# xingyizhou/CenterTrack

Measured on AMD Instinct MI355X. Metric: frames/sec (DLA-34 + DCNv2 CenterTrack hot path: H2D of the frame + forward + decode + D2H + track association), higher is better.
Workload: dtype f32; 1 GPU; mot17_512: mot heads, DLA-34, 512x512, 1 stream(s)/GPU, K=100, flip_test=False, seeded random-init weights; one step = 64 consecutive frames of every stream, each frame uploaded from pinned host memory inside the step (frame t+1 on a copy stream while frame t runs); global_batch=1, parallelism=streams sharded dp1, all-gather of packed detections, hip_graph=True

## Files before the change

### centertrack_amd/_lib.py

```python
import ctypes
import os

_PKG = os.path.dirname(os.path.abspath(__file__))
LIB_PATH = os.environ.get('CENTERTRACK_LIB') or os.path.join(_PKG, 'libcentertrack_hip.so')

c_float_p = ctypes.c_void_p
NUM_HEADS = 11
(HEAD_REG, HEAD_WH, HEAD_TRACKING, HEAD_LTRB, HEAD_LTRB_AMODAL, HEAD_DEP, HEAD_ROT, HEAD_DIM,
 HEAD_AMODEL_OFFSET, HEAD_NUSCENES_ATT, HEAD_VELOCITY) = range(NUM_HEADS)
HEAD_INDEX = {'reg': HEAD_REG, 'wh': HEAD_WH, 'tracking': HEAD_TRACKING, 'ltrb': HEAD_LTRB,
              'ltrb_amodal': HEAD_LTRB_AMODAL, 'dep': HEAD_DEP, 'rot': HEAD_ROT, 'dim': HEAD_DIM,
              'amodel_offset': HEAD_AMODEL_OFFSET, 'nuscenes_att': HEAD_NUSCENES_ATT,
              'velocity': HEAD_VELOCITY}
HEAD_CH = {'reg': 2, 'wh': 2, 'tracking': 2, 'ltrb': 4, 'ltrb_amodal': 4, 'dep': 1, 'rot': 8, 'dim': 3,
           'amodel_offset': 2, 'nuscenes_att': 8, 'velocity': 3}

CT_RELU = 1
CT_OUT_NCHW = 2
CT_DCN_MAIN, CT_DCN_FINISH, CT_DCN_OFFSETS = 1, 2, 4
CT_OK, CT_ERR_ARG, CT_ERR_LAUNCH, CT_ERR_WORKSPACE = 0, 1, 2, 3


class ConvDesc(ctypes.Structure):
    _fields_ = [('x', ctypes.c_void_p), ('N', ctypes.c_int), ('H', ctypes.c_int), ('W', ctypes.c_int),
                ('Cin', ctypes.c_int), ('ldx', ctypes.c_int),
                ('w_packed', ctypes.c_void_p), ('Cout', ctypes.c_int), ('ks', ctypes.c_int),
                ('stride', ctypes.c_int),
                ('scale', ctypes.c_void_p), ('shift', ctypes.c_void_p),
                ('res', ctypes.c_void_p), ('ldr', ctypes.c_int),
                ('y', ctypes.c_void_p), ('ldy', ctypes.c_int),
                ('flags', ctypes.c_int),
                ('sig_lo', ctypes.c_int), ('sig_hi', ctypes.c_int),
                ('dep_lo', ctypes.c_int), ('dep_hi', ctypes.c_int), ('depth_scale', ctypes.c_float),
                ('workspace', ctypes.c_void_p), ('workspace_bytes', ctypes.c_size_t),
                ('split_k', ctypes.c_int), ('algo', ctypes.c_int), ('w_winograd', ctypes.c_void_p),
                ('pool_y', ctypes.c_void_p), ('pool_ld', ctypes.c_int),
                ('proj_w_packed', ctypes.c_void_p), ('proj_scale', ctypes.c_void_p), ('proj_shift', ctypes.c_void_p),
                ('proj_y', ctypes.c_void_p), ('proj_ldy', ctypes.c_int)]


class DcnDesc(ctypes.Structure):
# ... 274 lines not shown
```

### centertrack_amd/build.py

```python
import os
import subprocess
import sys

PKG = os.path.dirname(os.path.abspath(__file__))
ROOT = os.path.dirname(PKG)
CSRC = os.path.join(PKG, 'csrc')
LIB = os.path.join(PKG, 'libcentertrack_hip.so')
SOURCES = ['api.cpp', 'runtime.hip', 'conv_mfma.hip', 'wino_mfma.hip', 'dcn_mfma.hip', 'stem.hip', 'elementwise.hip', 'decode.hip', 'pose.hip', 'host_track.cpp', 'host_preprocess.cpp', 'preprocess.hip', 'flip.hip', 'frame_loop.hip']
FLAGS = ['--offload-arch=gfx950', '-O3', '-std=c++17', '-fPIC', '-I' + os.path.join(ROOT, 'include'), '-I' + CSRC,
         '-Wno-unused-result']


def _stale(target, deps):
    if not os.path.exists(target):
        return True
    t = os.path.getmtime(target)
    return any(os.path.getmtime(d) > t for d in deps)


def build(force=False, verbose=False):
    hipcc = os.environ.get('HIPCC', '/opt/rocm/bin/hipcc')
    objdir = os.path.join(PKG, 'build')
    os.makedirs(objdir, exist_ok=True)
    headers = [os.path.join(CSRC, 'ct_common.h'), os.path.join(CSRC, 'ksplit_core.h'),
               os.path.join(ROOT, 'include', 'centertrack_hip.h')]
    objs = []
    procs = []
    for src in SOURCES:
        sp = os.path.join(CSRC, src)
        if not os.path.exists(sp):
            continue
        obj = os.path.join(objdir, src.rsplit('.', 1)[0] + '.o')
        objs.append(obj)
        if force or _stale(obj, [sp] + headers):
            extra = ['-x', 'hip'] if src.endswith('.hip') else ['-ffp-contract=off']
            cmd = [hipcc] + FLAGS + extra + ['-c', sp, '-o', obj]
            if verbose:
                print(' '.join(cmd))
            procs.append((src, subprocess.Popen(cmd)))
    for src, p in procs:
        if p.wait() != 0:
            raise RuntimeError('hipcc failed on %s' % src)
    if force or _stale(LIB, objs):
        cmd = [hipcc, '--offload-arch=gfx950', '-shared', '-fPIC', '-pthread', '-o', LIB] + objs
        if verbose:
            print(' '.join(cmd))
        subprocess.check_call(cmd)
# ... 6 lines not shown
```

### centertrack_amd/csrc/ct_common.h

```cpp
#pragma once
#include <hip/hip_runtime.h>
#include <stdint.h>
#include <stdio.h>

#include "centertrack_hip.h"

typedef float f32x4 __attribute__((ext_vector_type(4)));

void ct_set_error(const char *fmt, ...);

#define CT_FAIL_ARG(...)            \
    do {                            \
        ct_set_error(__VA_ARGS__);  \
        return CT_ERR_ARG;          \
    } while (0)

#define CT_CHECK_LAUNCH(name)                                              \
    do {                                                                   \
        hipError_t e__ = hipGetLastError();                                \
        if (e__ != hipSuccess) {                                           \
            ct_set_error("%s: launch failed: %s", name, hipGetErrorString(e__)); \
            return CT_ERR_LAUNCH;                                          \
        }                                                                  \
    } while (0)

static inline int ct_cdiv(int a, int b) { return (a + b - 1) / b; }

enum { CT_TUNE_CONV_CFG = 0, CT_TUNE_CONV_PIPE, CT_TUNE_CONV_SMALL_TILES, CT_TUNE_SPLITK_TARGET, CT_TUNE_DCN_BN,
       CT_TUNE_CONV_KS, CT_TUNE_CONV_KS_BELOW, CT_TUNE_CONV_KS_WAVES, CT_TUNE_XCD_REMAP, CT_TUNE_HEADS_ORDER, CT_TUNE_STEM_ROWS, CT_TUNE_DCN_SLOTS, CT_TUNE_DCN_XCD, CT_TUNE_COUNT };
int ct_tune_get(int key);
void ct_affine_inverse(const double *trans, double *M);
struct ct_wino_off_layer {
    const float *x; int N, H, W, Cin, ldx;
    const float *w_winograd;
    float *part;
};
int ct_wino_offsets_group(const ct_wino_off_layer *layers, int n, void *stream);

static inline int ct_xcd_per(int coutBlocks)
{
    return (ct_tune_get(CT_TUNE_XCD_REMAP) && coutBlocks >= 16 && (coutBlocks & 7) == 0) ? (coutBlocks >> 3) : 0;
}
#ifdef __HIPCC__
__device__ __forceinline__ int ct_block_cout(int &bid, int coutBlocks, int per)
{
    int cb;
    if (per) {
        const int j = bid >> 3;
        cb = (bid & 7) + 8 * (j % per);
        bid = j / per;
    } else {
        cb = bid % coutBlocks;
        bid /= coutBlocks;
    }
    return cb;
}
#endif

// ... 123 lines not shown
```

### centertrack_amd/csrc/dcn_mfma.hip

```cpp
#include <type_traits>

#include "ct_common.h"
#include "ksplit_core.h"

namespace {

struct DcnArgs {
    const float *x;
    const float *om;
    const float *wp;
    int N, H, W, Cin, ldx, ldom;
    int tilesX, tilesY, coutBlocks;
    int NT;
    int nchunks, chunksPerSplit;
    int tiles;
    int ptiles, splits;
    int xsx, xper, pband;
    float *ws;
    int wsCout;
    const float *w_off;
    const float *b_off;
    float *omPart;
    int omSplits;
    int offsOnly;
    EpiArgs epi;
};

constexpr int DCN_MAX_GROUP = 4;
struct DcnGroup {
    DcnArgs p[DCN_MAX_GROUP];
    int first[DCN_MAX_GROUP + 1];
    int n;
};

#ifndef CT_OFF_PD
#define CT_OFF_PD 2
#endif
CT_DEFINE_STAMPS(dcn)
#ifndef CT_ABL
#define CT_ABL 0
#endif
#ifndef CT_WS_AUX
#define CT_WS_AUX 0
#endif

__device__ __forceinline__ float dcn_mask_sigmoid(float v) { return __builtin_amdgcn_rcpf(1.0f + __expf(-v)); }

typedef float f32x2 __attribute__((ext_vector_type(2)));
__device__ __forceinline__ f32x4 dcn_blend(const f32x4 w, const f32x4 (&c)[4])
{
    const f32x2 w01 = w.lo, w23 = w.hi;
    f32x2 lo, hi;
    asm("v_pk_mul_f32 %0, %1, %2 op_sel_hi:[0,1]" : "=v"(lo) : "v"(w01), "v"(c[0].lo));
    asm("v_pk_mul_f32 %0, %1, %2 op_sel_hi:[0,1]" : "=v"(hi) : "v"(w01), "v"(c[0].hi));
    asm("v_pk_fma_f32 %0, %1, %2, %0 op_sel:[1,0,0] op_sel_hi:[1,1,1]" : "+v"(lo) : "v"(w01), "v"(c[1].lo));
    asm("v_pk_fma_f32 %0, %1, %2, %0 op_sel:[1,0,0] op_sel_hi:[1,1,1]" : "+v"(hi) : "v"(w01), "v"(c[1].hi));
    asm("v_pk_fma_f32 %0, %1, %2, %0 op_sel_hi:[0,1,1]" : "+v"(lo) : "v"(w23), "v"(c[2].lo));
    asm("v_pk_fma_f32 %0, %1, %2, %0 op_sel_hi:[0,1,1]" : "+v"(hi) : "v"(w23), "v"(c[2].hi));
    asm("v_pk_fma_f32 %0, %1, %2, %0 op_sel:[1,0,0] op_sel_hi:[1,1,1]" : "+v"(lo) : "v"(w23), "v"(c[3].lo));
    asm("v_pk_fma_f32 %0, %1, %2, %0 op_sel:[1,0,0] op_sel_hi:[1,1,1]" : "+v"(hi) : "v"(w23), "v"(c[3].hi));
    return f32x4{lo[0], lo[1], hi[0], hi[1]};
}

__device__ __forceinline__ void dcn_tab_entry(float dy, float dx, float mk, float fyk, float fxk, bool in, int H, int W, int ldx4,
                                              int rowb, int4 &o, f32x4 &w)
{
    const float ys = fyk + dy, xs = fxk + dx;
    const float yf = floorf(ys), xf = floorf(xs);
    const int y0 = (int)yf, x0 = (int)xf;
    const float ly = ys - yf, lx = xs - xf, hy = 1.0f - ly, hx = 1.0f - lx;
    const bool ok = in & (ys > -1.0f) & (xs > -1.0f) & (ys < (float)H) & (xs < (float)W);
    const bool vy0 = ok & (y0 >= 0), vy1 = ok & (y0 + 1 <= H - 1), vx0 = x0 >= 0, vx1 = x0 + 1 <= W - 1;
    const int base = __mul24(__mul24(y0, W) + x0, ldx4);
    o.x = (vy0 & vx0) ? base : 0;
    o.y = (vy0 & vx1) ? base + ldx4 : 0;
    o.z = (vy1 & vx0) ? base + rowb : 0;
    o.w = (vy1 & vx1) ? base + rowb + ldx4 : 0;
    w[0] = (vy0 & vx0) ? hy * hx * mk : 0.0f;
    w[1] = (vy0 & vx1) ? hy * lx * mk : 0.0f;
    w[2] = (vy1 & vx0) ? ly * hx * mk : 0.0f;
    w[3] = (vy1 & vx1) ? ly * lx * mk : 0.0f;
}

template <int WM, int WN>
__device__ __forceinline__ void dcn_store_acc(const DcnArgs &a, const f32x4 (&acc)[WM][WN], int n, int oy0, int ox0, int split, int nt0,
                                              int wm, int lane, const float (&psc)[WN], const float (&psh)[WN])
{
    const int li = lane & 15, lg = lane >> 4;
    if (a.ws) {
        const size_t Mtot = (size_t)a.N * a.H * a.W;
        float *wsp = a.ws + (size_t)split * Mtot * a.wsCout;
        const __amdgpu_buffer_rsrc_t srs = __builtin_amdgcn_make_buffer_rsrc(wsp, 0, (int)(Mtot * a.wsCout * 4), 0x00020000);
        const int pixb = a.wsCout * 4, rowb2 = a.W * pixb;
        const int oyb = oy0 + wm * WM;
        const int px0 = ox0 + lg * 4;
#pragma unroll
        for (int nt = 0; nt < WN; ++nt) {
            const int co = (nt0 + nt) * 16 + li;
            const int vbase = (((n * a.H + oyb) * a.W + px0) * a.wsCout + co) * 4;
            int vo[4];
#pragma unroll
            for (int e = 0; e < 4; ++e) vo[e] = (co < a.wsCout && px0 + e < a.W) ? vbase : (int)0x80000000;
#pragma unroll
            for (int mt = 0; mt < WM; ++mt) {
// ... 138 lines not shown
                b[kk][nt] = __builtin_bit_cast(f32x4, __builtin_amdgcn_raw_buffer_load_b128(wrs, bvo[nt], so + kk * slab_bytes, 0));
    };
    const int nsteps = (c_end - c_begin) * 9;
    const int nmax = nsteps;
    auto step_ct = [&](int st, int &chunk, int &tap) {
        const int u = min(max(st, 0), max(nsteps - 1, 0));
        const int c = u / 9;
        chunk = min(c_begin + c, nunits - 1);
        tap = u - c * 9;
    };
    f32x4 bq[2][NKK][WN];
    {
        int ch, tp;
        step_ct(0, ch, tp);
        load_b(bq[0], ch, tp);
    }
    float psc[WN], psh[WN];
#pragma unroll
    for (int nt = 0; nt < WN; ++nt) {
        psc[nt] = 1.0f; psh[nt] = 0.0f;
        if (!a.ws) ct_load_scale_shift(a.epi, (nt0 + nt) * 16, lane, psc[nt], psh[nt]);
    }

    {
        constexpr int E = BM * 9;
        constexpr int TI = (E + NTHR - 1) / NTHR;
        const int ldx4 = a.ldx * 4, rowb = a.W * ldx4;
        float tdy[TI], tdx[TI], tmk[TI];
        const int rot = (blockIdx.x >> 8) & 3;
        const int wrot = (wave - rot) & 3, trot = (tid - rot * 64) & 255;
#pragma unroll
        for (int i = 0; i < TI; ++i) {
            if (wrot * 64 + NTHR * i >= E) continue;
            const int it = trot + NTHR * i;
            const int k = it / BM, m = it & (BM - 1);
            const int oy = oy0 + (m >> 4), ox = ox0 + (m & 15);
            const bool in = it < E && oy < a.H && ox < a.W;
            if (parts) {
                const size_t plane = (size_t)a.N * a.H * a.W * 32;
                const float *pp = a.omPart + (in ? (((size_t)n * a.H + oy) * a.W + ox) * 32 : 0);
                const int kk = in ? k : 0;
                float dy = pp[2 * kk], dx = pp[2 * kk + 1], mk = pp[18 + kk];
                for (int sp = 1; sp < a.omSplits; ++sp) {
                    dy += pp[sp * plane + 2 * kk];
                    dx += pp[sp * plane + 2 * kk + 1];
                    mk += pp[sp * plane + 18 + kk];
// ... 432 lines not shown
    }
    CT_STAMP_VAL(17, nsteps);
    CT_STAMP_VAL(18, pi);
    CT_STAMP_RT(15);
}

}

extern "C" size_t ct_dcn_v2_offsets_bytes(const ct_dcn_desc *d)
{
    if (!d || (d->fuse_offset != 2 && d->fuse_offset != 3) || d->Cin % 64 || d->Cin <= 0 || d->N <= 0 || d->H <= 0 || d->W <= 0)
        return 0;
    return (size_t)(d->fuse_offset == 3 ? 1 : d->Cin / 64) * d->N * d->H * d->W * 32 * sizeof(float);
}

namespace {

struct DcnPlan {
    int fuse;
    int parts;
    int BM, BN, NKK, tilesX, tilesY, coutBlocks, NT, nchunks, splits, chunksPerSplit;
    int use_ws;
    int persist;
};

int make_plan(const ct_dcn_desc *d, DcnPlan *p, bool grouped)
{
    if (!d || !d->x || !d->w_packed || !d->y) CT_FAIL_ARG("ct_dcn_v2: null pointer");
    if (d->fuse_offset < 0 || d->fuse_offset > 3) CT_FAIL_ARG("ct_dcn_v2: fuse_offset=%d (0 .. 3)", d->fuse_offset);
    p->fuse = d->fuse_offset == 1;
    p->parts = d->fuse_offset == 2 ? d->Cin / 64 : (d->fuse_offset == 3 ? 1 : 0);
    if (d->fuse_offset && (!d->b_off || (d->fuse_offset != 3 && !d->w_off_packed && !(d->fuse_offset == 2 && d->w_off_winograd))))
        CT_FAIL_ARG("ct_dcn_v2: fuse_offset needs w_off_packed and b_off");
    if (d->fuse_offset && d->Cin % 64) CT_FAIL_ARG("ct_dcn_v2: fuse_offset needs Cin %% 64 == 0 (got %d)", d->Cin);
    if (p->parts) {
        const size_t need = ct_dcn_v2_offsets_bytes(d);
        if (!d->om_partial || d->om_partial_bytes < need) {
            ct_set_error("ct_dcn_v2: fuse_offset=%d needs %zu bytes of om_partial, got %zu", d->fuse_offset, need, d->om_partial ? d->om_partial_bytes : (size_t)0);
            return CT_ERR_WORKSPACE;
        }
    }
    if (!d->fuse_offset && !d->om) CT_FAIL_ARG("ct_dcn_v2: null offset/mask map");
    if (d->up_w) {
        if (!d->up_skip || !d->up_y) CT_FAIL_ARG("ct_dcn_v2: up_w given without up_skip / up_y");
        if (d->up_f != 2 && d->up_f != 4 && d->up_f != 8) CT_FAIL_ARG("ct_dcn_v2: up_f=%d unsupported", d->up_f);
        if (d->Cout % 4 || d->up_lds % 4 || d->up_ldy % 4 || ((uintptr_t)d->up_skip & 15) || ((uintptr_t)d->up_y & 15))
            CT_FAIL_ARG("ct_dcn_v2: up-sample views must be 16-byte aligned with Cout %% 4 == 0");
// ... 38 lines not shown
    }
    if (p->NKK == 4 && d->Cin % 64) CT_FAIL_ARG("ct_dcn_v2: the 64-channel-step shapes need Cin %% 64 == 0 (got %d)", d->Cin);
    p->tilesY = ct_cdiv(d->H, p->BM / 16);
    p->coutBlocks = ct_cdiv(d->Cout, p->BN);
    p->nchunks = d->Cin / 32;
    const long tiles = (long)d->N * p->tilesX * p->tilesY * p->coutBlocks;
    int splits = d->split_k;
    if (splits <= 0) {
        splits = 1;
        if (grouped) {
            splits = p->nchunks / 2;
        } else if (d->workspace && tiles < 256) {
            splits = (int)((512 + tiles - 1) / tiles);
            if (splits > 16) splits = 16;
        }
    }
    const int upc = p->NKK / 2;
    const int nunits = p->nchunks / upc;
    if (splits > nunits) splits = nunits;
    if (splits < 1) splits = 1;
    p->chunksPerSplit = ct_cdiv(nunits, splits) * upc;
    p->splits = ct_cdiv(p->nchunks, p->chunksPerSplit);
    p->use_ws = (p->splits > 1 || (grouped && d->up_w)) ? 1 : 0;
    if (p->persist) {
        const int ups = p->chunksPerSplit / upc;
        if (p->BM != 32 || (ups & 1) || nunits % ups)
            CT_FAIL_ARG("ct_dcn_v2: persistent shape needs an even number of %d-channel units per split (Cin=%d, split_k=%d)", 16 * p->NKK, d->Cin, p->splits);
        if ((double)d->N * d->H * d->W * d->ldx * 4.0 >= 4294967296.0) CT_FAIL_ARG("ct_dcn_v2: persistent shape: input view of 4 GiB or more");
    }
    return CT_OK;
}

size_t ws_bytes(const ct_dcn_desc *d, const DcnPlan &p)
{
    if (!p.use_ws) return 0;
    return (size_t)p.splits * d->N * d->H * d->W * (size_t)(p.NT * 16) * sizeof(float);
}

struct UpArgs {
    const float *w;
    const float *skip;
    float *y;
    int f, lds, ldy;
};
struct RedArgs {
    const float *ws;
    int splits, wsCout;
    size_t Mtot;
    int N, H, W;
    int rowBlocks;
    EpiArgs e;
    UpArgs u;
};
struct RedGroup {
    RedArgs p[DCN_MAX_GROUP];
    int first[DCN_MAX_GROUP + 1];
    int n;
};

// ... 55 lines not shown
        for (int jx = 0; jx < 2; ++jx) {
            const int xx = ix - jx;
            if (xx < 0 || xx >= W) continue;
            const unsigned m = ((unsigned)n * H + yy) * W + xx;
            const float *src = ws + (size_t)(m * wsCout + c);
            f32x4 s = *reinterpret_cast<const f32x4 *>(src);
            for (int k = 1; k < splits; ++k) s += *reinterpret_cast<const f32x4 *>(src + (size_t)k * plane);
            const int widx = (ky + f * jy) * kw + (kx + f * jx);
            const f32x4 wv = *reinterpret_cast<const f32x4 *>(u.w + widx * C + c);
#pragma unroll
            for (int i = 0; i < 4; ++i) acc[i] += ct_epilogue_value(e, s[i], c + i, sc[i], sh[i], 0.0f) * wv[i];
        }
    }
    *reinterpret_cast<f32x4 *>(u.y + (size_t)opix * u.ldy + c) = acc;
}

void fill_args(const ct_dcn_desc *d, const DcnPlan &p, DcnArgs *a)
{
    a->x = d->x; a->om = d->om; a->wp = d->w_packed;
    a->N = d->N; a->H = d->H; a->W = d->W; a->Cin = d->Cin; a->ldx = d->ldx; a->ldom = d->ldom;
    a->tilesX = p.tilesX; a->tilesY = p.tilesY; a->coutBlocks = p.coutBlocks; a->NT = p.NT;
    a->nchunks = p.nchunks; a->chunksPerSplit = p.chunksPerSplit;
    a->tiles = d->N * p.tilesX * p.tilesY * p.coutBlocks;
    a->ws = p.use_ws ? d->workspace : nullptr;
    a->wsCout = p.NT * 16;
    a->epi.scale = d->scale; a->epi.shift = d->shift; a->epi.res = nullptr; a->epi.y = d->y;
    a->epi.ldr = 0; a->epi.ldy = d->ldy; a->epi.Cout = d->Cout; a->epi.Ho = d->H; a->epi.Wo = d->W;
    a->epi.flags = d->flags & CT_RELU; a->epi.sig_lo = a->epi.sig_hi = 0; a->epi.dep_lo = a->epi.dep_hi = 0;
    a->epi.depth_scale = 1.0f;
    a->w_off = p.fuse ? d->w_off_packed : nullptr;
    a->b_off = d->fuse_offset ? d->b_off : nullptr;
    a->omPart = p.parts ? d->om_partial : nullptr;
    a->omSplits = p.parts;
    a->offsOnly = 0;
    a->ptiles = d->N * p.tilesX * p.tilesY;
    a->splits = p.splits;
    a->xsx = 0; a->xper = 0; a->pband = 0;
    if (ct_tune_get(CT_TUNE_DCN_XCD)) {
        int sx = 1;
        while (sx < 8 && p.splits % (2 * sx) == 0) sx *= 2;
        a->xsx = sx;
        a->pband = ct_cdiv(a->ptiles, 8 / sx);
        a->xper = p.coutBlocks * (p.splits / sx) * a->pband;
    }
}

size_t lds_bytes(int BM, bool fuse_any, bool single_chunk, int NKK = 2)
{
    using OffCfg = KsCfg<3, 1, 2, 2, 4>;
    size_t regionA = sizeof(float) * (size_t)(2 * NKK * BM * 16 + 2 * BM * 9 * 4);
    if (!fuse_any) return regionA;
    const size_t scratch = single_chunk ? sizeof(float) * (size_t)OffCfg::LDS1_FLOATS : OffCfg::LDS_BYTES;
    return sizeof(float) * (size_t)(BM * 32) + (scratch > regionA ? scratch : regionA);
}

int launch_group(const ct_dcn_desc *descs, int n, bool grouped, int phases, void *stream)
{
// ... 6 lines not shown
    long blocks = 0, rblocks = 0;
    bool fuse_any = false, single_chunk = true;
    const ct_dcn_desc *legacy_up = nullptr;
    for (int i = 0; i < n; ++i) {
        const ct_dcn_desc *d = descs + i;
        DcnPlan &p = plans[i];
        int rc = make_plan(d, &p, grouped);
        if (rc != CT_OK) return rc;
        if ((phases & CT_DCN_MAIN) && (p.BM != plans[0].BM || p.BN != plans[0].BN || p.NKK != plans[0].NKK || p.persist != plans[0].persist))
            CT_FAIL_ARG("ct_dcn_v2_group: layer %d resolves to another tile shape than layer 0", i);
        const size_t need = ws_bytes(d, p);
        if (need > 0 && (!d->workspace || d->workspace_bytes < need)) {
            ct_set_error("ct_dcn_v2: layer %d: split_k=%d needs %zu workspace bytes, got %zu", i, p.splits, need, d->workspace_bytes);
            return CT_ERR_WORKSPACE;
        }
        fill_args(d, p, &g.p[i]);
        fuse_any = fuse_any || p.fuse;
        if (p.fuse && d->Cin != 64) single_chunk = false;
        g.first[i] = (int)blocks;
        blocks += g.p[i].xsx ? 8L * g.p[i].xper : (long)g.p[i].tiles * p.splits;
        if (blocks > 0x7fffffffL) CT_FAIL_ARG("ct_dcn_v2: grid too large");
        if (p.use_ws) {
            RedArgs &r = rg.p[rg.n];
            r.ws = d->workspace; r.splits = p.splits; r.wsCout = g.p[i].wsCout;
            r.Mtot = (size_t)d->N * d->H * d->W;
            r.N = d->N; r.H = d->H; r.W = d->W;
            r.e = g.p[i].epi;
            long rows;
            if (d->up_w) {
                r.u.w = d->up_w; r.u.skip = d->up_skip; r.u.y = d->up_y; r.u.f = d->up_f; r.u.lds = d->up_lds; r.u.ldy = d->up_ldy;
                r.rowBlocks = (d->W * d->up_f * (d->Cout / 4) + 255) / 256;
                rows = (long)d->N * d->H * d->up_f;
            } else {
                r.u.w = nullptr; r.u.skip = nullptr; r.u.y = nullptr; r.u.f = 0; r.u.lds = r.u.ldy = 0;
                r.rowBlocks = (d->W * (r.wsCout / 4) + 255) / 256;
                rows = (long)d->N * d->H;
            }
            if ((double)r.Mtot * r.wsCout >= 1073741824.0 ||
                (d->up_w && (double)r.Mtot * d->up_f * d->up_f * (d->up_lds > d->up_ldy ? d->up_lds : d->up_ldy) >= 4294967296.0))
                CT_FAIL_ARG("ct_dcn_v2: layer %d: partial map / IDAUp output too large for the finishing launch", i);
            rg.first[rg.n] = (int)rblocks;
            rblocks += rows * r.rowBlocks;
            if (rblocks > 0x7fffffffL) CT_FAIL_ARG("ct_dcn_v2: grid too large");
            ++rg.n;
        } else if (d->up_w) {
            legacy_up = d;
        }
    }
    g.first[n] = (int)blocks;
    for (int i = n + 1; i <= DCN_MAX_GROUP; ++i) g.first[i] = (int)blocks;
    for (int i = n; i < DCN_MAX_GROUP; ++i) g.p[i] = g.p[0];
    const DcnPlan &p0 = plans[0];
    hipStream_t s = (hipStream_t)stream;
    if (phases & CT_DCN_OFFSETS) {
        DcnGroup og;
        og.n = 0;
        long oblocks = 0;
        ct_wino_off_layer wl[DCN_MAX_GROUP];
        int nw = 0;
        for (int i = 0; i < n; ++i) {
            const ct_dcn_desc *d = descs + i;
            if (d->fuse_offset != 2) continue;
            if (d->w_off_winograd) {
                ct_wino_off_layer &l = wl[nw++];
                l.x = d->x; l.N = d->N; l.H = d->H; l.W = d->W; l.Cin = d->Cin; l.ldx = d->ldx;
                l.w_winograd = d->w_off_winograd; l.part = d->om_partial;
                continue;
            }
            DcnArgs &a = og.p[og.n];
            a = g.p[i];
            a.tilesX = ct_cdiv(d->W, 16); a.tilesY = ct_cdiv(d->H, 2); a.coutBlocks = 1;
            a.tiles = d->N * a.tilesX * a.tilesY;
            a.w_off = d->w_off_packed;
            a.offsOnly = 1;
            og.first[og.n] = (int)oblocks;
            oblocks += (long)a.tiles * plans[i].parts;
            ++og.n;
        }
        if (og.n > 0) {
            if (oblocks > 0x7fffffffL) CT_FAIL_ARG("ct_dcn_v2: grid too large");
            for (int i = og.n; i <= DCN_MAX_GROUP; ++i) og.first[i] = (int)oblocks;
            for (int i = og.n; i < DCN_MAX_GROUP; ++i) og.p[i] = og.p[0];
            hipLaunchKernelGGL((dcn_mfma_kernel<32, 1, true>), dim3((unsigned)oblocks), dim3(256), lds_bytes(32, true, true), s, og);
            CT_CHECK_LAUNCH("ct_dcn_v2(offset/mask conv)");
        }
        if (nw > 0) {
            const int rc = ct_wino_offsets_group(wl, nw, stream);
            if (rc != CT_OK) return rc;
        }
// ... 135 lines not shown
```

### centertrack_amd/csrc/wino_mfma.hip

```cpp
#include "ct_common.h"

typedef unsigned u32x4 __attribute__((ext_vector_type(4)));

namespace {

struct WinoArgs {
    const float *x;
    const float *up;
    int N, H, W, Cin, ldx;
    int tilesX, tilesY, coutBlocks, xcdPer;
    int headMajor;
    int NT;
    int nchunks;
    EpiArgs epi;
    const float *hw2;
    const float *hb2;
    float *hout;
    int hctot;
    int hcout[CT_MAX_FUSED_HEADS], hcoff[CT_MAX_FUSED_HEADS];
};

template <int WM>
struct WCfg {
    static constexpr int PH = 4 * WM + 2, PW = 18, PP = PH * PW;
// ... 421 lines not shown
                    const float v = (hacc[h2][j] + hred[((q * 64 + lane) * 2 + h2) * 8 + j]) + a.hb2[cb * 8 + j];
                    a.hout[(((size_t)n * a.hctot + gc) * a.epi.Ho + oy) * a.epi.Wo + ox] =
                        ct_epilogue_value(a.epi, v, gc, 1.0f, 0.0f, 0.0f);
                }
            }
        }
    }
    if (HEADS) { CT_STAMP(6); CT_STAMP_RT(7); }
}

template <int WM, int WN, int KS, bool MULTI, int NB = 1, bool HEADS = false>
__global__ __launch_bounds__(256 * KS)
__attribute__((amdgpu_waves_per_eu(NB > 1 ? CT_NB_WAVES : ((!MULTI && KS == 1 && WM * WN <= 2) ? 4 : KS))))
void wino_conv_kernel(WinoArgs a)
{
    wino_body<WM, WN, KS, MULTI, NB, HEADS>(a, (int)blockIdx.x, gridDim.x, 0, a.epi.y);
}

struct WinoGroup {
    WinoArgs p[4];
    int first[5];
    int tiles[4];
    int sx[4], pband[4];
    int n;
};

__global__ __launch_bounds__(256) __attribute__((amdgpu_waves_per_eu(4))) void wino_offsets_kernel(WinoGroup g)
{
    int bid = blockIdx.x;
    int pi = 0;
#pragma unroll
    for (int i = 1; i < 4; ++i)
        if (i < g.n && bid >= g.first[i]) pi = i;
    const WinoArgs a = g.p[pi];
    bid -= g.first[pi];
    const int tiles = g.tiles[pi];
    const int sx = g.sx[pi], sper = (a.Cin >> 6) / sx;
    const int xcd = bid & 7;
    int j = bid >> 3;
    const int sh = j % sper; j /= sper;
    const int split = (xcd & (sx - 1)) + sx * sh;
    bid = (xcd / sx) * g.pband[pi] + j;
    if (j >= g.pband[pi] || bid >= tiles) return;
    float *ydst = a.epi.y + (size_t)split * a.N * a.H * a.W * 32;
    wino_body<1, 2, 1, false>(a, bid, (unsigned)tiles, split, ydst);
}

__global__ __launch_bounds__(256) void pack_winograd_kernel(const float *w, float *p, int Cout, int Cin, int NT)
{
    const size_t total = (size_t)16 * (Cin >> 4) * NT * 256;
    const size_t idx = (size_t)blockIdx.x * 256 + threadIdx.x;
    if (idx >= total) return;
    const int e = idx & 3, j = (idx >> 2) & 15, g = (idx >> 6) & 3;
    size_t t = idx >> 8;
    const int nt = t % NT; t /= NT;
    const int c16 = t % (Cin >> 4);
    const int pos = (int)(t / (Cin >> 4));
    const int co = nt * 16 + j, ci = c16 * 16 + 4 * g + e;
    float u = 0.0f;
    if (co < Cout) {
        const float G[4][3] = {{1.f, 0.f, 0.f}, {.5f, .5f, .5f}, {.5f, -.5f, .5f}, {0.f, 0.f, 1.f}};
        const int r = pos >> 2, c = pos & 3;
        const float *g3 = w + ((size_t)co * Cin + ci) * 9;
        for (int aa = 0; aa < 3; ++aa)
            for (int bb = 0; bb < 3; ++bb) u += G[r][aa] * g3[aa * 3 + bb] * G[c][bb];
    }
    p[idx] = u;
}
// ... 77 lines not shown
    return rc;
}

int ct_wino_offsets_group(const ct_wino_off_layer *L, int n, void *stream)
{
    if (n < 1 || n > 4) CT_FAIL_ARG("ct_wino_offsets_group: 1..4 layers");
    WinoGroup g;
    long blocks = 0;
    for (int i = 0; i < n; ++i) {
        const ct_wino_off_layer &l = L[i];
        if (!l.x || !l.w_winograd || !l.part || l.Cin % 64 || l.Cin <= 0 || l.ldx % 4 || ((uintptr_t)l.x & 15) || ((uintptr_t)l.part & 15))
            CT_FAIL_ARG("ct_wino_offsets_group: layer %d: bad arguments", i);
        WinoArgs &a = g.p[i];
        a.x = l.x; a.up = l.w_winograd;
        a.N = l.N; a.H = l.H; a.W = l.W; a.Cin = l.Cin; a.ldx = l.ldx;
        a.tilesX = ct_cdiv(l.W, 16); a.tilesY = ct_cdiv(l.H, 4); a.coutBlocks = 1; a.xcdPer = 0; a.headMajor = 0;
        a.NT = 2; a.nchunks = 1;
        a.epi.scale = nullptr; a.epi.shift = nullptr; a.epi.res = nullptr; a.epi.y = l.part;
        a.epi.ldr = 0; a.epi.ldy = 32; a.epi.Cout = 32; a.epi.Ho = l.H; a.epi.Wo = l.W;
        a.epi.flags = 0; a.epi.sig_lo = a.epi.sig_hi = 0; a.epi.dep_lo = a.epi.dep_hi = 0; a.epi.depth_scale = 1.0f;
        a.hw2 = nullptr; a.hb2 = nullptr; a.hout = nullptr; a.hctot = 0;
        for (int j = 0; j < CT_MAX_FUSED_HEADS; ++j) { a.hcout[j] = 0; a.hcoff[j] = 0; }
        g.tiles[i] = l.N * a.tilesX * a.tilesY;
        g.first[i] = (int)blocks;
        int sx = 1;
        while (sx < 8 && (l.Cin / 64) % (2 * sx) == 0) sx *= 2;
        g.sx[i] = sx;
        g.pband[i] = ct_cdiv(g.tiles[i], 8 / sx);
        blocks += 8L * (l.Cin / 64 / sx) * g.pband[i];
        if (blocks > 0x7fffffffL) CT_FAIL_ARG("ct_wino_offsets_group: grid too large");
    }
    for (int i = n; i <= 4; ++i) g.first[i] = (int)blocks;
    for (int i = n; i < 4; ++i) { g.p[i] = g.p[0]; g.tiles[i] = g.tiles[0]; g.sx[i] = g.sx[0]; g.pband[i] = g.pband[0]; }
    g.n = n;
    using C = WCfg<1>;
    const size_t patch = sizeof(float) * (size_t)C::BUF;
    const size_t exch = sizeof(float) * (size_t)(4 * 2 * 2 * 256 + 4 * 32 * 16);
    hipLaunchKernelGGL(wino_offsets_kernel, dim3((unsigned)blocks), dim3(256), patch > exch ? patch : exch, (hipStream_t)stream, g);
    CT_CHECK_LAUNCH("ct_dcn_v2(offset/mask convs, Winograd)");
    return CT_OK;
}

extern "C" int ct_heads_fused(const ct_heads_desc *d, void *stream)
{
    if (!d || !d->x || !d->w0_winograd || !d->b0 || !d->w2 || !d->b2 || !d->out) CT_FAIL_ARG("ct_heads_fused: null pointer");
    if (d->Cin != 64) CT_FAIL_ARG("ct_heads_fused: the heads read a 64-channel feature map (got %d)", d->Cin);
    if (d->ldx % 4 || ((uintptr_t)d->x & 15)) CT_FAIL_ARG("ct_heads_fused: input view must be 16-byte aligned");
    if (d->nheads < 1 || d->nheads > CT_MAX_FUSED_HEADS) CT_FAIL_ARG("ct_heads_fused: 1..%d heads", CT_MAX_FUSED_HEADS);
    if (d->N <= 0 || d->H <= 0 || d->W <= 0 || d->ctot <= 0) CT_FAIL_ARG("ct_heads_fused: bad shape");
    if (((uintptr_t)d->b0 & 15) || ((uintptr_t)d->w2 & 15)) CT_FAIL_ARG("ct_heads_fused: b0 / w2 must be 16-byte aligned");
    WinoArgs a;
    a.x = d->x; a.up = d->w0_winograd;
    a.N = d->N; a.H = d->H; a.W = d->W; a.Cin = 64; a.ldx = d->ldx;
    a.tilesX = ct_cdiv(d->W, 16); a.tilesY = ct_cdiv(d->H, 4); a.coutBlocks = d->nheads; a.xcdPer = 0;
    a.headMajor = ct_tune_get(CT_TUNE_HEADS_ORDER);
    a.NT = d->nheads * 16; a.nchunks = 1;
// ... 18 lines not shown
```

### centertrack_amd/model.py

```python
import ctypes
import os
from collections import OrderedDict

import torch

from . import _lib, autotune, ops
from .ops import View
from .weights import CHANNELS, LEVELS, dla34_param_shapes

BN_EPS = 1e-5
SMALL_SLOT_WGS = 600
FUSE_OFFSET = os.environ.get('CENTERTRACK_FUSE_OFFSET', '1') != '0'
WINOGRAD = os.environ.get('CENTERTRACK_WINOGRAD', '1') != '0'
FUSE_HEADS = os.environ.get('CENTERTRACK_FUSE_HEADS', '1') != '0'
FOLD_POOL = os.environ.get('CENTERTRACK_FOLD_POOL', '1') != '0'
FUSE_PROJ = os.environ.get('CENTERTRACK_FUSE_PROJ', '1') != '0'


def _fold_bn(sd, p):
    scale = sd[p + '.weight'].double() / torch.sqrt(sd[p + '.running_var'].double() + BN_EPS)
    shift = sd[p + '.bias'].double() - sd[p + '.running_mean'].double() * scale
    return scale.float().contiguous(), shift.float().contiguous()


# ... 492 lines not shown
                d = ops.make_conv_desc(ly.x, pk['w_off'], 27, 3, 1, out=omv, w_wino=pk['w_off_wino'])
                if tune:
                    autotune.tune_conv(d, dev)
                convs.setdefault(ly.main, []).append(
                    _Launch(ly.name + '.offset', 'conv', d, (ly.x, omv, pk),
                            ws_need=lib.ct_conv2d_workspace_bytes(ctypes.byref(d))))
            elif not ly.fused and split_offsets and ly.x.C % 64 == 0:
                part = torch.empty((ly.x.C // 64) * N * ly.x.H * ly.x.W * 32, dtype=torch.float32, device=dev)
                offs.setdefault(ly.main, []).append(ly)
            elif not ly.fused:
                om = ops.new_view(N, ly.x.H, ly.x.W, 32, dev)
                d = ops.make_conv_desc(ly.x, pk['w_off'], 27, 3, 1, shift=pk['b_off'], out=om, sig=(18, 27))
                if tune:
                    autotune.tune_conv(d, dev)
                convs.setdefault(ly.main, []).append(
                    _Launch(ly.name + '.offset', 'conv', d, (ly.x, om, pk),
                            ws_need=lib.ct_conv2d_workspace_bytes(ctypes.byref(d))))
            own = ly.fused or part is not None
            dd = ops.make_dcn_desc(ly.x, om, pk['w'], ly.cout, pk['scale'], pk['shift'], True, ly.out, up=ly.up,
                                   split_k=ly.splits, algo=3264, om_partial=part, raw_offsets=raw,
                                   w_off=pk['w_off'] if own else None, b_off=pk['b_off'] if own else None,
                                   w_off_wino=pk['w_off_wino'] if (split_offsets == 3 and not ly.fused) else None)
            need_c = ctypes.c_size_t(0)
            _lib.check(lib.ct_dcn_v2_group_plan(ctypes.byref(dd), ctypes.byref(need_c), None), 'DCN layer ' + ly.name)
            need = need_c.value
            ly.use_ws = need > 0
            keep = [ly.x, om, part, ly.out, pk, ly.up]
            if need:
                ws = torch.empty(need // 4, dtype=torch.float32, device=dev)
                dd.workspace, dd.workspace_bytes = ws.data_ptr(), need
                keep.append(ws)
            ly.desc = (dd, keep)
            if ly.use_ws:
                ly.finish = max(ly.main, (t_of(ly.up[2]) + 1) // 2) if ly.up is not None else ly.main
                done = 2 * ly.finish + 1
            else:
                ly.finish = None
                done = 2 * ly.main
            time_of[id((ly.up[3] if ly.up is not None else ly.out).buf)] = done
            slots.setdefault(ly.main, {'main': [], 'finish': []})['main'].append(ly)
            if ly.finish is not None:
                slots.setdefault(ly.finish, {'main': [], 'finish': []})['finish'].append(ly)
        out = []

        def group(lys, phases, tag):
            if phases == _lib.CT_DCN_MAIN:
                lys = sorted(lys, key=lambda ly: -((ly.x.C // 32 + ly.splits - 1) // ly.splits))
            for i in range(0, len(lys), 4):
                part = lys[i:i + 4]
                arr = (_lib.DcnDesc * len(part))()
                keep = []
                def can_persist(ly):
# ... 225 lines not shown
```

### include/centertrack_hip.h

```cpp
#ifndef CENTERTRACK_HIP_H
#define CENTERTRACK_HIP_H

#include <stddef.h>
#include <stdint.h>

#ifdef __cplusplus
extern "C" {
#endif

#define CT_OK 0
#define CT_ERR_ARG 1
#define CT_ERR_LAUNCH 2
#define CT_ERR_WORKSPACE 3

#define CT_RELU 1
#define CT_OUT_NCHW 2

#define CT_ABI_VERSION 103

const char *ct_last_error(void);
int ct_version(void);
int ct_set_tuning(const char *key, int value);

size_t ct_packed_weight_elems(int Cout, int Cin, int ks);
int ct_pack_conv_weight(const float *w_oihw, float *packed, int Cout, int Cin, int ks, void *stream);
size_t ct_packed_winograd_elems(int Cout, int Cin);
int ct_pack_winograd_weight(const float *w_oihw, float *packed, int Cout, int Cin, void *stream);

typedef struct ct_conv_desc {
    const float *x; int N, H, W, Cin, ldx;
    const float *w_packed; int Cout, ks, stride;
    const float *scale; const float *shift;
    const float *res; int ldr;
    float *y; int ldy;
    int flags;
    int sig_lo, sig_hi;
    int dep_lo, dep_hi; float depth_scale;
    float *workspace; size_t workspace_bytes;
    int split_k;
// ... 214 lines not shown
```

Before: 1167 frames/s.

## Build DCN sampling tables in the Winograd offset kernel's last split block

Adds an optional path, gated by a new CT_DCN_TABLES desc flag, in which the Winograd offset-conv kernel reduces the split partial offsets, adds the bias, applies the mask sigmoid and writes per-tile bilinear sampling tables (offsets and weights) into the DCN workspace. The last block per tile is elected with an atomic counter. The DCN main kernel (BM=32, non-persistent) then loads the precomputed table instead of recomputing sampling entries from the partials. This moves the table work out of every cout block of the DCN kernel, at the cost of extra workspace, atomics and fences. Nothing in the shown code sets the new flag, so the path may not run by default.

```diff
diff --git a/centertrack_amd/_lib.py b/centertrack_amd/_lib.py
--- a/centertrack_amd/_lib.py
+++ b/centertrack_amd/_lib.py
@@ -17,6 +17,7 @@
 
 CT_RELU = 1
 CT_OUT_NCHW = 2
+CT_DCN_TABLES = 4
 CT_DCN_MAIN, CT_DCN_FINISH, CT_DCN_OFFSETS = 1, 2, 4
 CT_OK, CT_ERR_ARG, CT_ERR_LAUNCH, CT_ERR_WORKSPACE = 0, 1, 2, 3
 
diff --git a/centertrack_amd/build.py b/centertrack_amd/build.py
--- a/centertrack_amd/build.py
+++ b/centertrack_amd/build.py
@@ -22,7 +22,7 @@
     hipcc = os.environ.get('HIPCC', '/opt/rocm/bin/hipcc')
     objdir = os.path.join(PKG, 'build')
     os.makedirs(objdir, exist_ok=True)
-    headers = [os.path.join(CSRC, 'ct_common.h'), os.path.join(CSRC, 'ksplit_core.h'),
+    headers = [os.path.join(CSRC, 'ct_common.h'), os.path.join(CSRC, 'ksplit_core.h'), os.path.join(CSRC, 'dcn_table.h'),
                os.path.join(ROOT, 'include', 'centertrack_hip.h')]
     objs = []
     procs = []
diff --git a/centertrack_amd/csrc/ct_common.h b/centertrack_amd/csrc/ct_common.h
--- a/centertrack_amd/csrc/ct_common.h
+++ b/centertrack_amd/csrc/ct_common.h
@@ -34,6 +34,9 @@
     const float *x; int N, H, W, Cin, ldx;
     const float *w_winograd;
     float *part;
+    const float *b_off;
+    char *tab;
+    unsigned *cnt;
 };
 int ct_wino_offsets_group(const ct_wino_off_layer *layers, int n, void *stream);
 
diff --git a/centertrack_amd/csrc/dcn_mfma.hip b/centertrack_amd/csrc/dcn_mfma.hip
--- a/centertrack_amd/csrc/dcn_mfma.hip
+++ b/centertrack_amd/csrc/dcn_mfma.hip
@@ -1,6 +1,7 @@
 #include <type_traits>
 
 #include "ct_common.h"
+#include "dcn_table.h"
 #include "ksplit_core.h"
 
 namespace {
@@ -23,6 +24,7 @@
     float *omPart;
     int omSplits;
     int offsOnly;
+    const char *tab;
     EpiArgs epi;
 };
 
@@ -43,8 +45,6 @@
 #ifndef CT_WS_AUX
 #define CT_WS_AUX 0
 #endif
-
-__device__ __forceinline__ float dcn_mask_sigmoid(float v) { return __builtin_amdgcn_rcpf(1.0f + __expf(-v)); }
 
 typedef float f32x2 __attribute__((ext_vector_type(2)));
 __device__ __forceinline__ f32x4 dcn_blend(const f32x4 w, const f32x4 (&c)[4])
@@ -60,26 +60,6 @@
     asm("v_pk_fma_f32 %0, %1, %2, %0 op_sel:[1,0,0] op_sel_hi:[1,1,1]" : "+v"(lo) : "v"(w23), "v"(c[3].lo));
     asm("v_pk_fma_f32 %0, %1, %2, %0 op_sel:[1,0,0] op_sel_hi:[1,1,1]" : "+v"(hi) : "v"(w23), "v"(c[3].hi));
     return f32x4{lo[0], lo[1], hi[0], hi[1]};
-}
-
-__device__ __forceinline__ void dcn_tab_entry(float dy, float dx, float mk, float fyk, float fxk, bool in, int H, int W, int ldx4,
-                                              int rowb, int4 &o, f32x4 &w)
-{
-    const float ys = fyk + dy, xs = fxk + dx;
-    const float yf = floorf(ys), xf = floorf(xs);
-    const int y0 = (int)yf, x0 = (int)xf;
-    const float ly = ys - yf, lx = xs - xf, hy = 1.0f - ly, hx = 1.0f - lx;
-    const bool ok = in & (ys > -1.0f) & (xs > -1.0f) & (ys < (float)H) & (xs < (float)W);
-    const bool vy0 = ok & (y0 >= 0), vy1 = ok & (y0 + 1 <= H - 1), vx0 = x0 >= 0, vx1 = x0 + 1 <= W - 1;
-    const int base = __mul24(__mul24(y0, W) + x0, ldx4);
-    o.x = (vy0 & vx0) ? base : 0;
-    o.y = (vy0 & vx1) ? base + ldx4 : 0;
-    o.z = (vy1 & vx0) ? base + rowb : 0;
-    o.w = (vy1 & vx1) ? base + rowb + ldx4 : 0;
-    w[0] = (vy0 & vx0) ? hy * hx * mk : 0.0f;
-    w[1] = (vy0 & vx1) ? hy * lx * mk : 0.0f;
-    w[2] = (vy1 & vx0) ? ly * hx * mk : 0.0f;
-    w[3] = (vy1 & vx1) ? ly * lx * mk : 0.0f;
 }
 
 template <int WM, int WN>
@@ -264,6 +244,19 @@
         if (!a.ws) ct_load_scale_shift(a.epi, (nt0 + nt) * 16, lane, psc[nt], psh[nt]);
     }
 
+    if (BM == 32 && a.tab) {
+        constexpr int NV = DCN_TAB_BYTES / 16, TV = (NV + NTHR - 1) / NTHR;
+        const int ptile = (n * a.tilesY + ty) * a.tilesX + tx;
+        const __amdgpu_buffer_rsrc_t trs = __builtin_amdgcn_make_buffer_rsrc(const_cast<char *>(a.tab), 0, a.ptiles * DCN_TAB_BYTES, 0x00020000);
+        f32x4 tv[TV];
+#pragma unroll
+        for (int i = 0; i < TV; ++i)
+            if (tid + i * NTHR < NV)
+                tv[i] = __builtin_bit_cast(f32x4, __builtin_amdgcn_raw_buffer_load_b128(trs, ptile * DCN_TAB_BYTES + (tid + i * NTHR) * 16, 0, 0));
+#pragma unroll
+        for (int i = 0; i < TV; ++i)
+            if (tid + i * NTHR < NV) *reinterpret_cast<f32x4 *>(reinterpret_cast<char *>(tab_off) + (tid + i * NTHR) * 16) = tv[i];
+    } else
     {
         constexpr int E = BM * 9;
         constexpr int TI = (E + NTHR - 1) / NTHR;
@@ -742,7 +735,16 @@
     int BM, BN, NKK, tilesX, tilesY, coutBlocks, NT, nchunks, splits, chunksPerSplit;
     int use_ws;
     int persist;
+    size_t tab_bytes;
+    int tab;
 };
+
+size_t tab_region_bytes(const ct_dcn_desc *d)
+{
+    const size_t tx = (size_t)ct_cdiv(d->W, 16);
+    const size_t bytes = (size_t)d->N * ct_cdiv(d->H, 2) * tx * DCN_TAB_BYTES + (size_t)d->N * ct_cdiv(d->H, 4) * tx * sizeof(unsigned);
+    return (bytes + 255) & ~(size_t)255;
+}
 
 int make_plan(const ct_dcn_desc *d, DcnPlan *p, bool grouped)
 {
@@ -827,6 +829,10 @@
     p->chunksPerSplit = ct_cdiv(nunits, splits) * upc;
     p->splits = ct_cdiv(p->nchunks, p->chunksPerSplit);
     p->use_ws = (p->splits > 1 || (grouped && d->up_w)) ? 1 : 0;
+    p->tab_bytes = (grouped && (d->flags & CT_DCN_TABLES) && d->fuse_offset == 2 && d->w_off_winograd) ? tab_region_bytes(d) : 0;
+    p->tab = (p->tab_bytes && p->BM == 32 && !p->persist) ? 1 : 0;
+    if (p->tab_bytes && (double)d->N * ct_cdiv(d->H, 2) * p->tilesX * DCN_TAB_BYTES >= 2147483648.0)
+        CT_FAIL_ARG("ct_dcn_v2: sampling tables of 2 GiB or more");
     if (p->persist) {
         const int ups = p->chunksPerSplit / upc;
         if (p->BM != 32 || (ups & 1) || nunits % ups)
@@ -838,8 +844,8 @@
 
 size_t ws_bytes(const ct_dcn_desc *d, const DcnPlan &p)
 {
-    if (!p.use_ws) return 0;
-    return (size_t)p.splits * d->N * d->H * d->W * (size_t)(p.NT * 16) * sizeof(float);
+    if (!p.use_ws) return p.tab_bytes;
+    return p.tab_bytes + (size_t)p.splits * d->N * d->H * d->W * (size_t)(p.NT * 16) * sizeof(float);
 }
 
 struct UpArgs {
@@ -941,7 +947,7 @@
     a->tilesX = p.tilesX; a->tilesY = p.tilesY; a->coutBlocks = p.coutBlocks; a->NT = p.NT;
     a->nchunks = p.nchunks; a->chunksPerSplit = p.chunksPerSplit;
     a->tiles = d->N * p.tilesX * p.tilesY * p.coutBlocks;
-    a->ws = p.use_ws ? d->workspace : nullptr;
+    a->ws = p.use_ws ? reinterpret_cast<float *>(reinterpret_cast<char *>(d->workspace) + p.tab_bytes) : nullptr;
     a->wsCout = p.NT * 16;
     a->epi.scale = d->scale; a->epi.shift = d->shift; a->epi.res = nullptr; a->epi.y = d->y;
     a->epi.ldr = 0; a->epi.ldy = d->ldy; a->epi.Cout = d->Cout; a->epi.Ho = d->H; a->epi.Wo = d->W;
@@ -952,6 +958,7 @@
     a->omPart = p.parts ? d->om_partial : nullptr;
     a->omSplits = p.parts;
     a->offsOnly = 0;
+    a->tab = p.tab ? reinterpret_cast<const char *>(d->workspace) : nullptr;
     a->ptiles = d->N * p.tilesX * p.tilesY;
     a->splits = p.splits;
     a->xsx = 0; a->xper = 0; a->pband = 0;
@@ -1004,7 +1011,7 @@
         if (blocks > 0x7fffffffL) CT_FAIL_ARG("ct_dcn_v2: grid too large");
         if (p.use_ws) {
             RedArgs &r = rg.p[rg.n];
-            r.ws = d->workspace; r.splits = p.splits; r.wsCout = g.p[i].wsCout;
+            r.ws = g.p[i].ws; r.splits = p.splits; r.wsCout = g.p[i].wsCout;
             r.Mtot = (size_t)d->N * d->H * d->W;
             r.N = d->N; r.H = d->H; r.W = d->W;
             r.e = g.p[i].epi;
@@ -1047,6 +1054,11 @@
                 ct_wino_off_layer &l = wl[nw++];
                 l.x = d->x; l.N = d->N; l.H = d->H; l.W = d->W; l.Cin = d->Cin; l.ldx = d->ldx;
                 l.w_winograd = d->w_off_winograd; l.part = d->om_partial;
+                l.b_off = d->b_off;
+                l.tab = plans[i].tab_bytes ? reinterpret_cast<char *>(d->workspace) : nullptr;
+                l.cnt = plans[i].tab_bytes ? reinterpret_cast<unsigned *>(reinterpret_cast<char *>(d->workspace) +
+                                                                          (size_t)d->N * ct_cdiv(d->H, 2) * ct_cdiv(d->W, 16) * DCN_TAB_BYTES)
+                                           : nullptr;
                 continue;
             }
             DcnArgs &a = og.p[og.n];
diff --git a/centertrack_amd/csrc/dcn_table.h b/centertrack_amd/csrc/dcn_table.h
--- /dev/null
+++ b/centertrack_amd/csrc/dcn_table.h
@@ -0,0 +1,27 @@
+#pragma once
+#include "ct_common.h"
+
+constexpr int DCN_TAB_ENTRIES = 32 * 9;
+constexpr int DCN_TAB_BYTES = DCN_TAB_ENTRIES * 32;
+
+__device__ __forceinline__ float dcn_mask_sigmoid(float v) { return __builtin_amdgcn_rcpf(1.0f + __expf(-v)); }
+
+__device__ __forceinline__ void dcn_tab_entry(float dy, float dx, float mk, float fyk, float fxk, bool in, int H, int W, int ldx4,
+                                              int rowb, int4 &o, f32x4 &w)
+{
+    const float ys = fyk + dy, xs = fxk + dx;
+    const float yf = floorf(ys), xf = floorf(xs);
+    const int y0 = (int)yf, x0 = (int)xf;
+    const float ly = ys - yf, lx = xs - xf, hy = 1.0f - ly, hx = 1.0f - lx;
+    const bool ok = in & (ys > -1.0f) & (xs > -1.0f) & (ys < (float)H) & (xs < (float)W);
+    const bool vy0 = ok & (y0 >= 0), vy1 = ok & (y0 + 1 <= H - 1), vx0 = x0 >= 0, vx1 = x0 + 1 <= W - 1;
+    const int base = __mul24(__mul24(y0, W) + x0, ldx4);
+    o.x = (vy0 & vx0) ? base : 0;
+    o.y = (vy0 & vx1) ? base + ldx4 : 0;
+    o.z = (vy1 & vx0) ? base + rowb : 0;
+    o.w = (vy1 & vx1) ? base + rowb + ldx4 : 0;
+    w[0] = (vy0 & vx0) ? hy * hx * mk : 0.0f;
+    w[1] = (vy0 & vx1) ? hy * lx * mk : 0.0f;
+    w[2] = (vy1 & vx0) ? ly * hx * mk : 0.0f;
+    w[3] = (vy1 & vx1) ? ly * lx * mk : 0.0f;
+}
diff --git a/centertrack_amd/csrc/wino_mfma.hip b/centertrack_amd/csrc/wino_mfma.hip
--- a/centertrack_amd/csrc/wino_mfma.hip
+++ b/centertrack_amd/csrc/wino_mfma.hip
@@ -1,4 +1,5 @@
 #include "ct_common.h"
+#include "dcn_table.h"
 
 typedef unsigned u32x4 __attribute__((ext_vector_type(4)));
 
@@ -467,8 +468,86 @@
     int first[5];
     int tiles[4];
     int sx[4], pband[4];
+    char *tab[4];
+    unsigned *cnt[4];
+    const float *b_off[4];
     int n;
 };
+
+__device__ __forceinline__ void wino_offsets_table(const WinoArgs &a, const float *b_off, char *tab, unsigned *cnt, int bid)
+{
+    extern __shared__ __attribute__((aligned(16))) float lds[];
+    const int tid = threadIdx.x;
+    const int S = a.Cin >> 6;
+    asm volatile("s_waitcnt vmcnt(0)" ::: "memory");
+    __syncthreads();
+    int *flag = reinterpret_cast<int *>(lds);
+    if (tid == 0) {
+        __builtin_amdgcn_fence(__ATOMIC_RELEASE, "agent");
+        asm volatile("s_waitcnt vmcnt(0)" ::: "memory");
+        const unsigned old = atomicAdd(cnt + bid, 1u);
+        const int last = old == (unsigned)(S - 1);
+        if (last) {
+            atomicExch(cnt + bid, 0u);
+            __builtin_amdgcn_fence(__ATOMIC_ACQUIRE, "agent");
+            asm volatile("s_waitcnt vmcnt(0)" ::: "memory");
+        }
+        *flag = last;
+    }
+    __syncthreads();
+    if (!*flag) return;
+
+    const int tx = bid % a.tilesX;
+    const int ty4 = (bid / a.tilesX) % a.tilesY;
+    const int n = bid / (a.tilesX * a.tilesY);
+    const int H = a.H, W = a.W, tilesY2 = (H + 1) >> 1;
+    const int ldx4 = a.ldx * 4, rowb = W * ldx4;
+    const size_t plane = (size_t)a.N * H * W * 32;
+    const float *part = a.epi.y;
+    constexpr int SB = 8;
+    const __amdgpu_buffer_rsrc_t trs = __builtin_amdgcn_make_buffer_rsrc(tab, 0, a.N * tilesY2 * a.tilesX * DCN_TAB_BYTES, 0x00020000);
+#pragma unroll
+    for (int i = 0; i < 3; ++i) {
+        const int e = tid + 256 * i;
+        const int h = e >= DCN_TAB_ENTRIES ? 1 : 0;
+        const int ty2 = ty4 * 2 + h;
+        if (e >= 2 * DCN_TAB_ENTRIES || ty2 >= tilesY2) continue;
+        const int it = e - h * DCN_TAB_ENTRIES, k = it >> 5, m = it & 31;
+        const int ky = (k * 11) >> 5, kx = k - 3 * ky;
+        const int oy = ty2 * 2 + (m >> 4), ox = tx * 16 + (m & 15);
+        const bool in = oy < H && ox < W;
+        float dy = 0.0f, dx = 0.0f, mk = 0.0f;
+        if (in) {
+            const float *pp = part + (((size_t)n * H + oy) * W + ox) * 32;
+            for (int s0 = 0; s0 < S; s0 += SB) {
+                float v[SB][3];
+#pragma unroll
+                for (int j = 0; j < SB; ++j) {
+                    if (s0 + j >= S) break;
+                    const float *q = pp + (size_t)(s0 + j) * plane;
+                    v[j][0] = q[2 * k];
+                    v[j][1] = q[2 * k + 1];
+                    v[j][2] = q[18 + k];
+                }
+#pragma unroll
+                for (int j = 0; j < SB; ++j) {
+                    if (s0 + j >= S) break;
+                    if (s0 + j == 0) { dy = v[j][0]; dx = v[j][1]; mk = v[j][2]; }
+                    else { dy += v[j][0]; dx += v[j][1]; mk += v[j][2]; }
+                }
+            }
+            dy += b_off[2 * k];
+            dx += b_off[2 * k + 1];
+            mk = dcn_mask_sigmoid(mk + b_off[18 + k]);
+        }
+        int4 o;
+        f32x4 w;
+        dcn_tab_entry(dy, dx, mk, (float)(oy - 1 + ky), (float)(ox - 1 + kx), in, H, W, ldx4, rowb, o, w);
+        const int vo = ((n * tilesY2 + ty2) * a.tilesX + tx) * DCN_TAB_BYTES + it * 16;
+        __builtin_amdgcn_raw_buffer_store_b128(__builtin_bit_cast(u32x4, o), trs, vo, 0, 0);
+        __builtin_amdgcn_raw_buffer_store_b128(__builtin_bit_cast(u32x4, w), trs, vo + DCN_TAB_ENTRIES * 16, 0, 0);
+    }
+}
 
 __global__ __launch_bounds__(256) __attribute__((amdgpu_waves_per_eu(4))) void wino_offsets_kernel(WinoGroup g)
 {
@@ -489,6 +568,7 @@
     if (j >= g.pband[pi] || bid >= tiles) return;
     float *ydst = a.epi.y + (size_t)split * a.N * a.H * a.W * 32;
     wino_body<1, 2, 1, false>(a, bid, (unsigned)tiles, split, ydst);
+    if (g.tab[pi]) wino_offsets_table(a, g.b_off[pi], g.tab[pi], g.cnt[pi], bid);
 }
 
 __global__ __launch_bounds__(256) void pack_winograd_kernel(const float *w, float *p, int Cout, int Cin, int NT)
@@ -612,6 +692,9 @@
         a.hw2 = nullptr; a.hb2 = nullptr; a.hout = nullptr; a.hctot = 0;
         for (int j = 0; j < CT_MAX_FUSED_HEADS; ++j) { a.hcout[j] = 0; a.hcoff[j] = 0; }
         g.tiles[i] = l.N * a.tilesX * a.tilesY;
+        g.tab[i] = l.tab; g.cnt[i] = l.cnt; g.b_off[i] = l.b_off;
+        if (l.tab && (!l.cnt || !l.b_off || ((uintptr_t)l.tab & 15)))
+            CT_FAIL_ARG("ct_wino_offsets_group: layer %d: sampling tables need counters, the bias and 16-byte alignment", i);
         g.first[i] = (int)blocks;
         int sx = 1;
         while (sx < 8 && (l.Cin / 64) % (2 * sx) == 0) sx *= 2;
@@ -621,7 +704,10 @@
         if (blocks > 0x7fffffffL) CT_FAIL_ARG("ct_wino_offsets_group: grid too large");
     }
     for (int i = n; i <= 4; ++i) g.first[i] = (int)blocks;
-    for (int i = n; i < 4; ++i) { g.p[i] = g.p[0]; g.tiles[i] = g.tiles[0]; g.sx[i] = g.sx[0]; g.pband[i] = g.pband[0]; }
+    for (int i = n; i < 4; ++i) {
+        g.p[i] = g.p[0]; g.tiles[i] = g.tiles[0]; g.sx[i] = g.sx[0]; g.pband[i] = g.pband[0];
+        g.tab[i] = g.tab[0]; g.cnt[i] = g.cnt[0]; g.b_off[i] = g.b_off[0];
+    }
     g.n = n;
     using C = WCfg<1>;
     const size_t patch = sizeof(float) * (size_t)C::BUF;
diff --git a/centertrack_amd/model.py b/centertrack_amd/model.py
--- a/centertrack_amd/model.py
+++ b/centertrack_amd/model.py
@@ -538,12 +538,13 @@
                                    w_off=pk['w_off'] if own else None, b_off=pk['b_off'] if own else None,
                                    w_off_wino=pk['w_off_wino'] if (split_offsets == 3 and not ly.fused) else None)
             need_c = ctypes.c_size_t(0)
-            _lib.check(lib.ct_dcn_v2_group_plan(ctypes.byref(dd), ctypes.byref(need_c), None), 'DCN layer ' + ly.name)
+            splits_c = ctypes.c_int(0)
+            _lib.check(lib.ct_dcn_v2_group_plan(ctypes.byref(dd), ctypes.byref(need_c), ctypes.byref(splits_c)), 'DCN layer ' + ly.name)
             need = need_c.value
-            ly.use_ws = need > 0
+            ly.use_ws = splits_c.value > 1 or ly.up is not None
             keep = [ly.x, om, part, ly.out, pk, ly.up]
             if need:
-                ws = torch.empty(need // 4, dtype=torch.float32, device=dev)
+                ws = torch.zeros(need // 4, dtype=torch.float32, device=dev)
                 dd.workspace, dd.workspace_bytes = ws.data_ptr(), need
                 keep.append(ws)
             ly.desc = (dd, keep)
diff --git a/include/centertrack_hip.h b/include/centertrack_hip.h
--- a/include/centertrack_hip.h
+++ b/include/centertrack_hip.h
@@ -15,6 +15,7 @@
 
 #define CT_RELU 1
 #define CT_OUT_NCHW 2
+#define CT_DCN_TABLES 4
 
 #define CT_ABI_VERSION 103
 
```

After: 1154 frames/s, median of 2. 0.988x the previous value.
